# ecrireme/ESR-NeRF

Hardware: AMD Instinct MI355X
Metric: training rays/sec at 4096 rays x 128 samples (fine stage) (higher is better)
Workload: dtype f32; 1 GPU; C2: giftbox_w fine stage on the slab scene, 4096 rays x 128 samples per GPU, grid 256x256x64, s_val=20, forward + trainer loss + backward + the TV lines on every third step (no optimizer step); rays_per_gpu=4096, samples_per_ray=128, surviving_samples=524288, parallelism=dp1

## Files before the change

### esr_nerf_amd/_lib.py

```python
from __future__ import annotations

import ctypes as C
import os

import torch

_HERE = os.path.dirname(os.path.abspath(__file__))
LIB_PATH = os.path.join(_HERE, "libesr_hip.so")
LIB_PATH = os.environ.get("ESR_LIB_PATH", LIB_PATH)
ABI_VERSION = 30
_lib = None


class EsrScene(C.Structure):
    _fields_ = [
        ("xyz_min", C.c_float * 3), ("xyz_max", C.c_float * 3),
        ("mask_min", C.c_float * 3), ("mask_max", C.c_float * 3),
        ("gx", C.c_int32), ("gy", C.c_int32), ("gz", C.c_int32),
        ("mx", C.c_int32), ("my", C.c_int32), ("mz", C.c_int32),
        ("near_", C.c_float), ("stepdist", C.c_float), ("voxel_size", C.c_float),
        ("act_shift", C.c_float), ("mask_thres", C.c_float), ("fast_thres", C.c_float),
        ("s_val", C.c_float), ("max_steps", C.c_int32), ("grad_feat", C.c_float * 4),
    ]


class EsrPlan(C.Structure):
    _fields_ = [(n, C.c_int32) for n in
                ("n_on", "n_off", "tiles_on", "tiles_all", "m0", "m1", "m2", "overflow")]


class EsrFeatArgs(C.Structure):
    _fields_ = [(n, C.c_void_p) for n in ("rays_o", "rays_d", "viewdirs", "rec_ray", "rec_step", "rec_sdf",
                                          "pts", "pt_viewdirs", "pt_sdf")] + \
# ... 79 lines not shown
    _fields_ = [("w", C.c_void_p * 4), ("b", C.c_void_p * 4)]


class EsrWgradJob(C.Structure):
    _fields_ = [("kind", C.c_int32), ("color_row0", C.c_int32), ("t0", C.c_int32), ("t1", C.c_int32),
                ("X", C.c_void_p), ("H", C.c_void_p), ("dZ", C.c_void_p), ("dz", C.c_void_p),
                ("gw", C.c_void_p), ("gb", C.c_void_p), ("X16", C.c_void_p), ("amax", C.c_void_p)]


EXPORTS = [
    "esr_abi_version", "esr_build_info",
    "esr_sample_count", "esr_sample_fill", "esr_alpha2weight_fwd", "esr_alpha2weight_bwd",
    "esr_tv_add_grad", "esr_segment_sum",
    "esr_sample_count_f64", "esr_sample_fill_f64", "esr_alpha2weight_fwd_f64", "esr_alpha2weight_bwd_f64",
    "esr_infer_t_minmax", "esr_infer_n_samples", "esr_infer_ray_start_dir", "esr_sample_ndc_pts", "esr_sample_bg_pts",
    "esr_maskcache_lookup", "esr_raw2alpha", "esr_raw2alpha_bwd", "esr_tv_add_grad_masked",
    "esr_fine_march_count", "esr_fine_plan_begin", "esr_fine_plan", "esr_fine_plan_totals", "esr_fine_plan_offsets", "esr_fine_march_fill",
    "esr_fine_march_bwd", "esr_fine_march_bwd_rec", "esr_fine_march_cache_floats", "esr_fine_march_count_cached",
    "esr_fine_march_fill_cached", "esr_fine_march_bwd_cached", "esr_fine_march_count_ga", "esr_fine_march_fill_ga", "esr_fine_march_bwd_ga",
    "esr_fine_feat_fwd", "esr_fine_feat_fwd_x16", "esr_fine_feat_x16_bytes", "esr_fine_feat_bwd",
    "esr_mlp_packed_floats", "esr_mlp_pack", "esr_mlp_pack_batch", "esr_mlp_packed_split_elems", "esr_mlp_split_gain_offset", "esr_mlp_split_range_flag", "esr_mlp_fwd_split", "esr_mlp_fwd_fine_split", "esr_mlp_dgrad_split", "esr_mlp_dgrad_fine_split", "esr_absmax", "esr_mlp_fwd", "esr_mlp_fwd_mixed", "esr_mlp_fwd_fine", "esr_mlp_dgrad_fine", "esr_mlp_fwd_fine_bf16", "esr_mlp_dgrad_fine_bf16", "esr_mlp_dgrad", "esr_mlp_wgrad", "esr_mlp_wgrad_batch", "esr_tone_wgrad_scratch_floats", "esr_tone_wgrad_recompute", "esr_tone_wgrad_recompute_bf16", "esr_tone_wgrad_recompute_split",
    "esr_mlp_wgrad_scratch_floats",
    "esr_fine_tone_in_fwd", "esr_fine_composite_fwd", "esr_fine_composite_bwd",
    "esr_fine_tone_in_bwd", "esr_fine_loss_fwd_bwd_dp",
    "esr_expgrad_fwd", "esr_expgrad_bwd", "esr_lts_dirs", "esr_lts_ref_order", "esr_lts_perturb", "esr_lts_gather_rows",
    "esr_lts_gather_points", "esr_lts_combine_fwd", "esr_lts_combine_bwd",
    "esr_act_fwd", "esr_act_bwd", "esr_act_batch", "esr_lts_gather_rows_batch", "esr_pair_loss_batch", "esr_lts_ref_order_inv", "esr_lts_dirs_rays", "esr_composite3_fwd", "esr_composite3_bwd", "esr_lts_tone_in_bwd",
    "esr_sample_points", "esr_pair_loss_fwd_bwd", "esr_emit_edit",
    "esr_gauss3d_fwd", "esr_gauss3d_bwd", "esr_central_grad_fwd", "esr_central_grad_bwd",
    "esr_coarse_march_count", "esr_coarse_march_fill", "esr_coarse_march_bwd", "esr_coarse_march_count_ga", "esr_coarse_march_fill_ga", "esr_coarse_march_bwd_ga",
    "esr_coarse_feat_fwd", "esr_coarse_feat_bwd", "esr_coarse_shade_fwd", "esr_coarse_shade_bwd",
    "esr_adam_step", "esr_eval_aux", "esr_eval_disp",
    "esr_mlp_packed_bf16_elems", "esr_mlp_pack_bf16", "esr_mlp_fwd_bf16", "esr_mlp_dgrad_bf16", "esr_mlp_wgrad_bf16",
    "esr_brick_floats", "esr_brick_flags", "esr_brick_pack", "esr_brick_unpack", "esr_brick_list", "esr_brick_list_scratch_ints",
    "esr_smooth_grad_tv_fwd", "esr_smooth_grad_tv_bwd", "esr_host_choice_noreplace", "esr_host_choice_start", "esr_host_choice_wait",
    "esr_mesh_field", "esr_mesh_blocks", "esr_mesh_count", "esr_mesh_emit",
    "esr_cd_sample_count", "esr_cd_sample_fill", "esr_cd_cell_keys", "esr_cd_hash_insert", "esr_cd_downsample_round",
    "esr_cd_nn",
    "esr_dvgo_fwd", "esr_dvgo_eval", "esr_dvgo_bwd", "esr_dvgo_count", "esr_dvgo_count_add",
    "esr_ssim", "esr_view_post", "esr_sqerr_sum", "esr_gamma_curve", "esr_mask_iou",
    "esr_mask_dilate", "esr_edit_label",
]

SIGNATURES = {
    "esr_mask_dilate": (C.c_int, [C.c_void_p, C.c_int32, C.c_int32, C.c_int32, C.c_int32, C.c_void_p, C.c_void_p]),
    "esr_edit_label": (C.c_int, [C.c_void_p, C.c_int64, C.c_void_p, C.c_float, C.c_int32, C.c_int32, C.c_void_p, C.c_int32,
                                 C.c_void_p, C.c_void_p, C.c_void_p, C.c_void_p, C.c_void_p, C.c_void_p, C.c_void_p,
                                 C.c_void_p, C.c_void_p]),
}


def lib() -> C.CDLL:
    global _lib
    if _lib is None:
        if not os.path.exists(LIB_PATH):
            raise RuntimeError(
                f"{LIB_PATH} is missing: build it with `python -m esr_nerf_amd.build` "
                "(there is no CPU fallback for the HIP path)")
        L = C.CDLL(LIB_PATH)
        L.esr_abi_version.restype = C.c_int
        L.esr_build_info.restype = C.c_char_p
        if hasattr(L, "esr_mlp_packed_floats"):
            L.esr_mlp_packed_floats.restype = C.c_int64
            L.esr_mlp_wgrad_scratch_floats.restype = C.c_int64
            L.esr_tone_wgrad_scratch_floats.restype = C.c_int64
            L.esr_fine_march_cache_floats.restype = C.c_int64
        if hasattr(L, "esr_fine_feat_x16_bytes"):
            L.esr_fine_feat_x16_bytes.restype = C.c_int64
        if hasattr(L, "esr_brick_list_scratch_ints"):
            L.esr_brick_list_scratch_ints.restype = C.c_int64
        if hasattr(L, "esr_mlp_packed_bf16_elems"):
# ... 60 lines not shown
```

### esr_nerf_amd/csrc/shade.hip

```cpp
#include "esr_common.h"

namespace {

constexpr int XT_ROWS = 48;

__device__ __forceinline__ float softplus_grad(float z) { return z > 20.f ? 1.f : esr_sigmoid(z); }

__global__ void __launch_bounds__(256) tone_in_fwd_kernel(const float *__restrict__ z_off,
                                                          const float *__restrict__ z_emo, int tiles_on,
                                                          int tiles_all, float *__restrict__ lin,
                                                          float *__restrict__ Xt)
{
    const int total = tiles_all * 32;
    for (int j = blockIdx.x * blockDim.x + threadIdx.x; j < total; j += gridDim.x * blockDim.x) {
        const int t = j >> 5, s = j & 31;
        const size_t z4 = (size_t)t * 4 * 32 + s;
        float *X = Xt + (size_t)t * XT_ROWS * 32 + s;
#pragma unroll
        for (int c = 0; c < 3; ++c) {
            float v = esr_softplus(z_off[z4 + c * 32]);
            if (t < tiles_on) v = esr_softplus(z_emo[z4 + c * 32]) + v;
            lin[z4 + c * 32] = v;
            X[c * 32] = v;
#pragma unroll
// ... 109 lines not shown
            if (ray >= 0) {
                d = rec_w[j] * g_lin[3 * ray + c] + dX[c * 32];
#pragma unroll
                for (int i = 0; i < 5; ++i) {
                    const float f = (float)(1 << i);
                    d += f * (dX[(3 + c * 5 + i) * 32] * X[(18 + c * 5 + i) * 32] - dX[(18 + c * 5 + i) * 32] * X[(3 + c * 5 + i) * 32]);
                }
                const float z = (t < tiles_on) ? z_emo[z4 + c * 32] : z_off[z4 + c * 32];
                d *= softplus_grad(z);
            }
            dz[z4 + c * 32] = d;
        }
        dz[z4 + 96] = 0.f;
    }
}

__device__ __forceinline__ float wave_sum(float v)
{
#pragma unroll
    for (int off = 32; off > 0; off >>= 1) v += __shfl_xor(v, off);
    return v;
}

__global__ void __launch_bounds__(256) loss_kernel(const float *__restrict__ srgb_m,
                                                   const float *__restrict__ lin_m,
                                                   const float *__restrict__ last,
                                                   const float *__restrict__ rgbs, int n_rays, float white_bg,
                                                   float w_lin, float w_ent, float scale, float *__restrict__ loss,
                                                   float *__restrict__ g_srgb, float *__restrict__ g_lin,
                                                   float *__restrict__ g_last)
{
    const float inv = scale == 1.f ? 1.f / (3.f * (float)n_rays) : scale / (3.f * (float)n_rays);
    w_ent *= scale;
    float acc = 0.f;
    for (int r = blockIdx.x * blockDim.x + threadIdx.x; r < n_rays; r += gridDim.x * blockDim.x) {
        const float al = last[r];
        const float bg = al * white_bg;
        float gl = 0.f;
#pragma unroll
        for (int c = 0; c < 3; ++c) {
            const float gt = rgbs[3 * r + c];
            const float ps = srgb_m[3 * r + c] + bg;
            const float xs = fminf(fmaxf(ps, 0.f), 1.f);
            acc += (xs - gt) * (xs - gt) * inv;
            const float gs = (ps >= 0.f && ps <= 1.f) ? 2.f * (xs - gt) * inv : 0.f;
            g_srgb[3 * r + c] = gs;
            const float pl = lin_m[3 * r + c] + bg;
            const float l0 = fmaxf(pl, 0.f);
            const bool sat = gt >= 1.f;
            const float x = sat ? fminf(l0, 1.f) : l0;
            const bool low = x <= 0.0031308f;
            const float y = low ? 12.92f * x : 1.055f * powf(x, 1.f / 2.4f) - 0.055f;
            acc += w_lin * (y - gt) * (y - gt) * inv;
            float g = w_lin * 2.f * (y - gt) * inv;
            g *= low ? 12.92f : 1.055f * (1.f / 2.4f) * powf(x, 1.f / 2.4f - 1.f);
            if (sat && !(l0 <= 1.f)) g = 0.f;
            if (!(pl >= 0.f)) g = 0.f;
            g_lin[3 * r + c] = g;
            gl += (gs + g) * white_bg;
        }
        if (r == n_rays - 1) {
            const float p = fminf(fmaxf(al, 1e-6f), 1.f - 1e-6f);
            acc += w_ent * -(p * logf(p) + (1.f - p) * logf(1.f - p));
            if (al >= 1e-6f && al <= 1.f - 1e-6f) gl += w_ent * -(logf(p) - logf(1.f - p));
        }
        g_last[r] = gl;
    }
    acc = wave_sum(acc);
    if (esr_lane() == 0 && acc != 0.f) atomicAdd(loss, acc);
}

__global__ void __launch_bounds__(256) pair_loss_kernel(const float *__restrict__ a, const float *__restrict__ b,
                                                        int64_t rows, int cols, const uint8_t *__restrict__ row_mask,
                                                        int mask_value, const int32_t *__restrict__ count_dev, int kind,
                                                        float w_value, float w_a, float w_b, float *__restrict__ loss,
                                                        float *__restrict__ ga, float *__restrict__ gb)
{
    const int64_t total = rows * cols;
    const int64_t n_sel = count_dev ? (int64_t)count_dev[0] * cols : total;
    const float inv = n_sel > 0 ? 1.f / (float)n_sel : 0.f;
    float acc = 0.f;
    for (int64_t i = blockIdx.x * (int64_t)blockDim.x + threadIdx.x; i < total; i += (int64_t)gridDim.x * blockDim.x) {
        const bool sel = !row_mask || (int)row_mask[i / cols] == mask_value;
        float g = 0.f;
        if (sel) {
            const float d = a[i] - (b ? b[i] : 0.f);
            if (kind == 0) { acc += d * d * inv; g = 2.f * d * inv; }
            else { acc += fabsf(d) * inv; g = (d > 0.f ? 1.f : (d < 0.f ? -1.f : 0.f)) * inv; }
        }
        if (ga) ga[i] = w_a * g;
        if (gb) gb[i] = -w_b * g;
    }
// ... 292 lines not shown
    if (!dXt || !Xt || !g_lin || !lin || !z_off || (tiles_on && !z_emo) || !rec_ray || !rec_w || !dz) return ESR_EINVAL;
    tone_in_bwd_kernel<<<esr_grid_for((int64_t)tiles_all * 32, 256), 256, 0, esr_stream(stream)>>>(
        dXt, Xt, g_lin, lin, z_off, z_emo, rec_ray, rec_w, tiles_on, tiles_all, dz);
    ESR_CHECK_LAUNCH();
    return 0;
}

ESR_API int esr_fine_loss_fwd_bwd_dp(const float *srgb_marched, const float *lin_marched,
                                     const float *alphainv_last, const float *rgbs, int32_t n_rays,
                                     float white_bg, float weight_linear, float weight_entropy_last, float scale,
                                     float *loss, float *g_srgb, float *g_lin, float *g_last, void *stream)
{
    if (n_rays < 0) return ESR_EINVAL;
    if (n_rays == 0) return 0;
    if (!srgb_marched || !lin_marched || !alphainv_last || !rgbs || !loss || !g_srgb || !g_lin || !g_last)
        return ESR_EINVAL;
    loss_kernel<<<esr_grid_for(n_rays, 256), 256, 0, esr_stream(stream)>>>(
        srgb_marched, lin_marched, alphainv_last, rgbs, n_rays, white_bg, weight_linear,
        weight_entropy_last, scale, loss, g_srgb, g_lin, g_last);
    ESR_CHECK_LAUNCH();
    return 0;
}

ESR_API int esr_eval_aux(const float *X, int32_t xrows, int32_t row_nx, int32_t row_ny, int32_t row_nz,
                         const int32_t *rec_ray, const int32_t *rec_step, int32_t tiles,
                         const float *pos_rt_host, float stepdist, float *aux, void *stream)
{
    if (tiles < 0 || xrows < 1 || row_nx < 0 || row_ny < 0 || row_nz < 0 || row_nx >= xrows || row_ny >= xrows ||
        row_nz >= xrows)
        return ESR_EINVAL;
    if (tiles == 0) return 0;
    if (!X || !rec_ray || !rec_step || !pos_rt_host || !aux) return ESR_EINVAL;
    EvalAux A = {};
    A.X = X; A.rec_ray = rec_ray; A.rec_step = rec_step; A.tiles = tiles; A.xrows = xrows; A.stepdist = stepdist;
    A.aux = aux; A.nrow[0] = row_nx; A.nrow[1] = row_ny; A.nrow[2] = row_nz;
    for (int i = 0; i < 9; ++i) A.rt[i] = pos_rt_host[i];
    eval_aux_kernel<<<esr_grid_for((int64_t)tiles * 32, 256), 256, 0, esr_stream(stream)>>>(A);
    ESR_CHECK_LAUNCH();
    return 0;
}

ESR_API int esr_eval_disp(const float *depth3, const float *alphainv_last, float far_, int32_t n_rays,
                          float *depth, float *disp, void *stream)
{
    if (n_rays < 0) return ESR_EINVAL;
    if (n_rays == 0) return 0;
// ... 143 lines not shown
```

### esr_nerf_amd/fine_engine.py

```python
from __future__ import annotations

import ctypes as C
import functools
import math
import os
from dataclasses import dataclass
from typing import Dict, List, Optional

import torch

from . import _lib

KIND_RADIANCE, KIND_TONEMAP = 0, 1
HID = 192
X_ROWS, DX_ROWS, XT_ROWS = 104, 64, 48


def make_scene(xyz_min, xyz_max, mask_min, mask_max, world_size, mask_size, near, stepdist,
               voxel_size, act_shift, mask_thres, fast_thres, s_val, grad_feat) -> _lib.EsrScene:
    sc = _lib.EsrScene()
    for i in range(3):
        sc.xyz_min[i], sc.xyz_max[i] = float(xyz_min[i]), float(xyz_max[i])
        sc.mask_min[i], sc.mask_max[i] = float(mask_min[i]), float(mask_max[i])
    sc.gx, sc.gy, sc.gz = [int(v) for v in world_size]
# ... 20 lines not shown
    n: int
    rays_o: torch.Tensor
    rays_d: torch.Tensor
    viewdirs: Optional[torch.Tensor]
    mask_density: torch.Tensor
    sdf: torch.Tensor
    cnt3: torch.Tensor
    off3: torch.Tensor
    stats: torch.Tensor
    last: torch.Tensor
    cache: Optional[torch.Tensor] = None
    tiles_on: int = 0
    tiles_all: int = 0
    counts: Dict[str, int] = None
    e_pre: object = None


@dataclass
class FineCtx:
    march: March
    feat_args: object = None
    x16: bool = False
    f32_only: bool = False
    counts = property(lambda self: self.march.counts)


FINE_ROWS = dict(X=X_ROWS, gnorm=4, H0=HID, H1=HID, H2=HID, z_off=4, z_emo=4, lin=4, Xt=XT_ROWS, Ht=HID,
                 zt=4, rgb=4, dzt=4, dZt=HID, dXt=DX_ROWS, dz=4, dZ0=HID, dZ1=HID, dZ2=HID, dX=DX_ROWS,
                 dweight=1, rec_w=1, rec_sdf=1, dsdf=1)
FINE_OTHER = dict(M0=(192, torch.int32), M1=(192, torch.int32), M2=(192, torch.int32), Mt=(192, torch.int32),
                  rec_ray=(32, torch.int32), rec_step=(32, torch.int32), X16=(26 * 256, torch.uint8))


class _Workspace:
    min_tiles = 0

    def __init__(self, device, rows=FINE_ROWS, other=FINE_OTHER):
        self.device, self.rows, self.other = device, rows, other
        self.cap_tiles = 0
        self.buf: Dict[str, torch.Tensor] = {}
        self.ray_bufs: Dict[int, Dict[str, torch.Tensor]] = {}
        self.cache = None

    def ensure(self, tiles: int):
        if tiles <= self.cap_tiles:
            return
# ... 58 lines not shown

class FineEngine:
    def __init__(self, device, mlp_dtype: str = "f32"):
        if mlp_dtype not in ("f32", "bf16"):
            raise ValueError("mlp_dtype must be 'f32' or 'bf16'")
        self.device = torch.device(device)
        self.bf16 = mlp_dtype == "bf16"
        self.packed16: Dict[str, torch.Tensor] = {}
        self._p16: Dict[int, C.c_void_p] = {}
        self.L = _lib.lib()
        self.ws = _Workspace(self.device)
        self.plan_dev = torch.zeros(8, dtype=torch.int32, device=self.device)
        self.plan_host = torch.zeros(8, dtype=torch.int32).pin_memory()
        self.packed = {
            k: torch.empty(self.L.esr_mlp_packed_floats(kind), dtype=torch.float32, device=self.device)
            for k, kind in (("off", KIND_RADIANCE), ("emo", KIND_RADIANCE), ("tone", KIND_TONEMAP))}
        self.wgrad_scratch = torch.empty(self.L.esr_mlp_wgrad_scratch_floats(), dtype=torch.float32,
                                         device=self.device)
        self._timing = False
        self._only = None
        self._events = []
        self.n_calls = 0
        self.overlap_wgrad = True
        self._side = None
        self._raw: Dict[str, tuple] = {}
        self._pack_cache: Dict[str, tuple] = {}
        self._pack_pending = None
        self._pack_batch_cache = None
        self.x16 = self.bf16
        self.split_fwd = (not self.bf16) and os.environ.get("ESR_SPLIT_FWD", "1") != "0"
        self.split_strict = os.environ.get("ESR_SPLIT_STRICT", "0") == "1"
        self.split_fallback_steps = 0
        self.packed_split: Dict[str, torch.Tensor] = {}
        self._psplit = {}
        self.range_flag = None
        self._range_host = None
        self._range_event = None
        if self.split_fwd:
            key = str(self.device)
            if key not in _RANGE_FLAGS:
                _RANGE_FLAGS[key] = torch.zeros(1, dtype=torch.int32, device=self.device)
            self.range_flag = _RANGE_FLAGS[key]
            self._range_host = torch.zeros(1, dtype=torch.int32).pin_memory()
            with torch.cuda.device(self.device):
                _lib.check(self.L.esr_mlp_split_range_flag(_lib.ptr(self.range_flag)), "esr_mlp_split_range_flag")
        self.tone_scratch = torch.empty(self.L.esr_tone_wgrad_scratch_floats(), dtype=torch.float32, device=self.device)
# ... 263 lines not shown
        return _lib.ptr_array([self.ws[n] for n in names])

    def feat_args(self, m: March, rec, color_on, color_off):
        fa = _lib.EsrFeatArgs()
        fa.rays_o, fa.rays_d, fa.viewdirs = m.rays_o.data_ptr(), m.rays_d.data_ptr(), m.viewdirs.data_ptr()
        fa.rec_ray, fa.rec_step, fa.rec_sdf = rec[0].data_ptr(), rec[1].data_ptr(), rec[3].data_ptr()
        fa.sdf = m.sdf.data_ptr()
        for g in range(3):
            fa.color_on[g] = color_on[g].data_ptr() if color_on[g] is not None else None
            fa.color_off[g] = color_off[g].data_ptr() if color_off[g] is not None else None
        fa.tiles_on, fa.tiles_all = m.tiles_on, m.tiles_all
        return fa

    def _tone_wgrad(self, x, dz, t0, t1, gw, gb, amax, s, name):
        (w0, w1), (b0, _) = self._raw["tone"]
        L = self.L
        fn = L.esr_tone_wgrad_recompute_split if amax is not None else \
            L.esr_tone_wgrad_recompute_bf16 if self.bf16 else L.esr_tone_wgrad_recompute
        self._run(name, fn, _lib.ptr(x), _lib.ptr(dz), _lib.ptr(w0.detach()), _lib.ptr(b0.detach()), _lib.ptr(w1.detach()),
                  *((_lib.ptr(amax),) if amax is not None else ()), t0, t1, _lib.ptr(gw[0]), _lib.ptr(gb[0]), _lib.ptr(gw[1]),
                  _lib.ptr(gb[1]), _lib.ptr(self.tone_scratch), C.c_int64(self.tone_scratch.numel()), s)

    def forward(self, scene, rays_o, rays_d, viewdirs, em_modes, mask_density, sdf, off_color, emo_color, prelude=None,
                heal: bool = True):
        run = lambda: self._forward(scene, rays_o, rays_d, viewdirs, em_modes, mask_density, sdf, off_color, emo_color, prelude)
        return self.healed(run) if heal else run()

    def _forward(self, scene, rays_o, rays_d, viewdirs, em_modes, mask_density, sdf, off_color, emo_color, prelude=None):
        L, s, ws = self.L, self._s(), self.ws
        n = rays_o.shape[0]
        for t in (rays_o, rays_d, viewdirs):
            if t.dtype != torch.float32:
                raise RuntimeError("rays must be fp32")
        if em_modes.dtype != torch.int64:
            raise RuntimeError("em_modes must be int64")
        n3 = (3 * n + 3) // 4 * 4
        zb = torch.zeros(8 + 2 * n3 + 4, dtype=torch.float32, device=self.device)
        plan_dev = zb[:8].view(torch.int32)
        srgb, lin = zb[8: 8 + 3 * n].view(n, 3), zb[8 + n3: 8 + n3 + 3 * n].view(n, 3)
        self._loss_acc = zb[8 + 2 * n3: 8 + 2 * n3 + 2]
        self._amax = zb[8 + 2 * n3 + 3: 8 + 2 * n3 + 4]
        self._amax_t = zb[8 + 2 * n3 + 2: 8 + 2 * n3 + 3]
        sp = C.byref(scene)
        main = torch.cuda.current_stream(self.device)
        m = self._march_plan(ws, scene, rays_o, rays_d, viewdirs, em_modes, mask_density, sdf, plan_dev=plan_dev, prelude=prelude)
        last, e_pre, tiles_on, tiles_all = m.last, m.e_pre, m.tiles_on, m.tiles_all
        ctx = FineCtx(march=m, f32_only=not self.bf16 and not self.split_fwd)
        if tiles_all == 0:
            if e_pre is not None:
                main.wait_event(e_pre)
            self.range_probe()
# ... 8 lines not shown
        else:
            self._run("feat_fwd", L.esr_fine_feat_fwd, sp, C.byref(fa), _lib.ptr(ws["X"]), _lib.ptr(ws["gnorm"]), s)
        ctx.feat_args = fa
        H, M = self._H(["H0", "H1", "H2"]), self._H(["M0", "M1", "M2"])
        if e_pre is not None:
            main.wait_event(e_pre)
        if not self.bf16 and self.split_fwd and "off" in self.packed_split and "emo" in self.packed_split:
            self._run("mlp_fwd(rad)", L.esr_mlp_fwd_fine_split, _lib.ptr(self.packed["off"]), _lib.ptr(self.packed_split["off"]),
                      _lib.ptr(self.packed["emo"]), _lib.ptr(self.packed_split["emo"]), _lib.ptr(ws["X"]), tiles_on, tiles_all,
                      H, M, 88, _lib.ptr(ws["z_off"]), _lib.ptr(ws["z_emo"]), s)
        elif not self.bf16:
            self._run("mlp_fwd(rad)", L.esr_mlp_fwd_fine, _lib.ptr(self.packed["off"]), _lib.ptr(self.packed["emo"]),
                      _lib.ptr(ws["X"]), tiles_on, tiles_all, H, M, 88, _lib.ptr(ws["z_off"]), _lib.ptr(ws["z_emo"]), s)
        else:
            po, pe = _lib.ptr(self.packed["off"]), _lib.ptr(self.packed["emo"])
            self._run("mlp_fwd(rad)", L.esr_mlp_fwd_fine_bf16, po, self._p16[po.value], pe, self._p16[pe.value], _lib.ptr(ws["X"]),
                      _lib.ptr(ws["X16"]) if x16 else None, tiles_on, tiles_all, H, M, 88, _lib.ptr(ws["z_off"]),
                      _lib.ptr(ws["z_emo"]), s)
        self._run("tone_in_fwd", L.esr_fine_tone_in_fwd, _lib.ptr(ws["z_off"]), _lib.ptr(ws["z_emo"]), tiles_on, tiles_all,
                                          _lib.ptr(ws["lin"]), _lib.ptr(ws["Xt"]), s)
        self._run("mlp_fwd(tone)", self.mlp_fwd, KIND_TONEMAP, _lib.ptr(self.packed["tone"]), _lib.ptr(ws["Xt"]), 0, tiles_all,
                                 self._H(["Ht"]), self._H(["Mt"]), 2, 0, _lib.ptr(ws["zt"]), s)
        self.range_probe()
        self._run("composite_fwd", L.esr_fine_composite_fwd, _lib.ptr(ws["zt"]), _lib.ptr(ws["lin"]), _lib.ptr(ws["rec_ray"]),
                                            _lib.ptr(ws["rec_w"]), tiles_all, _lib.ptr(ws["rgb"]),
                                            _lib.ptr(srgb), _lib.ptr(lin), s)
        return ctx, last, srgb, lin

    @torch.no_grad()
    def evaluate(self, *args):
        return self.healed(lambda: self._evaluate(*args))

    def _evaluate(self, scene, rays_o, rays_d, viewdirs, mask_density, sdf, off_color, emo_color, pos_rt, far,
                  em_mode: int):
        L, s, ws, dev = self.L, self._s(), self.ws, self.device
        n = rays_o.shape[0]
        em0 = torch.zeros(n, dtype=torch.int64, device=dev)
        m = self._march_plan(ws, scene, rays_o, rays_d, viewdirs, em0, mask_density, sdf)
        T = m.tiles_all
        z3 = lambda: torch.zeros(n, 3, dtype=torch.float32, device=dev)
        out = {f"{sp_}/{v}_rgb": z3() for v in ("off", "on", "emo") for sp_ in ("srgb", "lin")}
        if T:
            sp = C.byref(scene)
            fa = self.feat_args(m, ws.rec(), color_on=(None, None, None), color_off=(off_color, emo_color, None))
            self._run("feat_fwd", L.esr_fine_feat_fwd, sp, C.byref(fa), _lib.ptr(ws["X"]), _lib.ptr(ws["gnorm"]), s)
            H, M = self._H(["H0", "H1", "H2"]), self._H(["M0", "M1", "M2"])
# ... 78 lines not shown
            todo = [(KIND_RADIANCE, ws["X"], Hh, dZh, ws["dz"], 0, to, "emo_w", "emo_b"),
                    (KIND_RADIANCE, ws["X"], Hh, dZh, ws["dz"], to, ta, "off_w", "off_b")]
            jobs = (_lib.EsrWgradJob * len(todo))()
            for j, (kind, X, Hs, dZs, dzs, r0, r1, gwk, gbk) in enumerate(todo):
                gwa, gba = _lib.ptr_array(grads[gwk]), _lib.ptr_array(grads[gbk])
                keep += [gwa, gba]
                jb = jobs[j]
                jb.kind, jb.color_row0, jb.t0, jb.t1 = kind, 0, r0, r1
                jb.X, jb.dz = X.data_ptr(), dzs.data_ptr()
                jb.H, jb.dZ = C.addressof(Hs), C.addressof(dZs)
                jb.gw, jb.gb = C.addressof(gwa), C.addressof(gba)
                if ctx.x16:
                    jb.X16 = ws["X16"].data_ptr()
                if split:
                    jb.amax = ctx.amax.data_ptr()
            self._run("mlp_wgrad(all)", L.esr_mlp_wgrad_batch, jobs, len(todo), 1 if self.bf16 else 0,
                      _lib.ptr(self.wgrad_scratch), C.c_int64(self.wgrad_scratch.numel()), s_)

        if ta == 0:
            march_bwd(s)
            if after_grids is not None:
                after_grids()
            return
        self._run("composite_bwd", L.esr_fine_composite_bwd, _lib.ptr(g_srgb), _lib.ptr(g_lin), _lib.ptr(ws["rgb"]),
                  _lib.ptr(ws["lin"]), _lib.ptr(ws["rec_ray"]), _lib.ptr(ws["rec_w"]), ta, _lib.ptr(ws["dweight"]),
                  _lib.ptr(ws["dzt"]), s)
        if fold:
            march_bwd(s)
        dZt_arg = _lib.ptr_array([None])
        M = self._H(["M0", "M1", "M2"])
        dZ = self._H(["dZ0", "dZ1", "dZ2"])
        if self.bf16:
            self._run("mlp_dgrad(tone)", L.esr_mlp_dgrad_bf16, KIND_TONEMAP, self._p16[self.packed["tone"].data_ptr()],
                      _lib.ptr(ws["dzt"]), 0, ta, self._H(["Mt"]), dZt_arg, _lib.ptr(ws["dXt"]), s)
        elif split:
            self._run("mlp_dgrad(tone)", L.esr_mlp_dgrad_split, KIND_TONEMAP, _lib.ptr(self.packed_split["tone"]), _lib.ptr(ws["dzt"]),
                      0, ta, self._H(["Mt"]), dZt_arg, _lib.ptr(ws["dXt"]), _lib.ptr(ctx.amax_t), s)
        else:
            self._run("mlp_dgrad(tone)", L.esr_mlp_dgrad, KIND_TONEMAP, _lib.ptr(self.packed["tone"]), _lib.ptr(ws["dzt"]), 0, ta,
                      self._H(["Mt"]), dZt_arg, _lib.ptr(ws["dXt"]), s)
        self._run("tone_in_bwd", L.esr_fine_tone_in_bwd, _lib.ptr(ws["dXt"]), _lib.ptr(ws["Xt"]), _lib.ptr(g_lin), _lib.ptr(ws["lin"]),
                  _lib.ptr(ws["z_off"]), _lib.ptr(ws["z_emo"]), _lib.ptr(ws["rec_ray"]), _lib.ptr(ws["rec_w"]), to, ta,
                  _lib.ptr(ws["dz"]), s)
        if self.bf16:
            pe, po = self.packed["emo"].data_ptr(), self.packed["off"].data_ptr()
            self._run("mlp_dgrad(rad)", L.esr_mlp_dgrad_fine_bf16, self._p16[pe], self._p16[po],
                      _lib.ptr(ws["dz"]), to, ta, M, dZ, _lib.ptr(ws["dX"]), s)
        elif split:
            self._run("mlp_dgrad(rad)", L.esr_mlp_dgrad_fine_split, _lib.ptr(self.packed_split["emo"]),
                      _lib.ptr(self.packed_split["off"]), _lib.ptr(ws["dz"]), to, ta, M, dZ, _lib.ptr(ws["dX"]),
                      _lib.ptr(ctx.amax), s)
        else:
            self._run("mlp_dgrad(rad)", L.esr_mlp_dgrad_fine, _lib.ptr(self.packed["emo"]), _lib.ptr(self.packed["off"]),
                      _lib.ptr(ws["dz"]), to, ta, M, dZ, _lib.ptr(ws["dX"]), s)
        if not overlap:
            feat_bwd(s)
            if not fold:
                march_bwd(s)
            if after_grids is not None:
                after_grids()
            wgrads(s)
            return
        e_dgrad = torch.cuda.Event()
        e_dgrad.record(main)
        side = self._side_stream(0)
        side.wait_event(e_dgrad)
        with torch.cuda.stream(side):
            wgrads(_lib.stream_ptr(self.device))
            e_w = torch.cuda.Event()
            e_w.record(side)
        feat_bwd(s)
        if not fold:
            march_bwd(s)
        if after_grids is not None:
            after_grids()
        main.wait_event(e_w)

    def _side_stream(self, i=0):
        if self._side is None:
            self._side = {}
        if i not in self._side:
            self._side[i] = torch.cuda.Stream(self.device)
        return self._side[i]

    def loss_fwd_bwd(self, last, srgb, lin, rgbs, white_bg=True, weight_linear=0.1, weight_entropy_last=0.001,
                     scale=1.0):
        n = last.shape[0]
        acc = getattr(self, "_loss_acc", None)
        self._loss_acc = None
        pair = acc if acc is not None and acc.device == srgb.device else torch.zeros(2, dtype=torch.float32, device=self.device)
        self.loss_pair = pair
        loss = pair[:1]
        g_srgb = torch.empty_like(srgb)
        g_lin = torch.empty_like(lin)
        g_last = torch.empty_like(last)
        self._run("loss", self.L.esr_fine_loss_fwd_bwd_dp,
                  _lib.ptr(srgb), _lib.ptr(lin), _lib.ptr(last), _lib.ptr(rgbs.contiguous()), n,
                  C.c_float(1.0 if white_bg else 0.0), C.c_float(weight_linear), C.c_float(weight_entropy_last),
                  C.c_float(scale), _lib.ptr(loss), _lib.ptr(g_srgb), _lib.ptr(g_lin), _lib.ptr(g_last), self._s())
        return loss, g_last, g_srgb, g_lin
```

### esr_nerf_amd/trainer.py

```python
from __future__ import annotations

import os

from typing import Dict, Optional, Tuple

import torch

from .fine_engine import KIND_RADIANCE, KIND_TONEMAP


def shard_batch(batch: Dict[str, torch.Tensor], rank: int, world: int) -> Dict[str, torch.Tensor]:
    n = next(iter(batch.values())).shape[0]
    per = n // world
    lo = rank * per
    hi = n if rank == world - 1 else lo + per
    return {k: v[lo:hi].contiguous() for k, v in batch.items()}


def dp_loss_weights(n_local: int, global_rays, entropy_owner: bool, weight_entropy_last: float):
    scale = 1.0 if global_rays is None else n_local / float(global_rays)
    w_ent = (weight_entropy_last / scale) if entropy_owner else 0.0
    return scale, w_ent


# ... 250 lines not shown
                              global_rays: Optional[int] = None,
                              entropy_owner: bool = True,
                              regularisers: Optional[dict] = None) -> Tuple[torch.Tensor, Dict[str, torch.Tensor]]:
        m = self.model
        eng = m.engine
        m.s_val = s_val
        ps = m._mlp_params()
        return self._step(eng, lambda _: self._attempt(batch, global_rays, entropy_owner, m, eng, ps, regularisers))

    def _attempt(self, batch, global_rays, entropy_owner, m, eng, ps, regularisers):
        g = None

        def prelude():
            nonlocal g
            with eng.packing():
                eng.pack("off", KIND_RADIANCE, list(ps[0:8:2]), list(ps[1:8:2]))
                eng.pack("emo", KIND_RADIANCE, list(ps[8:16:2]), list(ps[9:16:2]))
                eng.pack("tone", KIND_TONEMAP, list(ps[16:20:2]), list(ps[17:20:2]))
            g = self._alloc_grads(batch["rays_o"].device)

        ctx, last, srgb, lin = eng.forward(
            m.scene_struct(), batch["rays_o"], batch["rays_d"], batch["viewdirs"], batch["em_modes"],
            m.mask_cache.density.view(*m.mask_cache.density.shape[2:]),
            m.sdf.device_view(), m.off_color.device_view(), m.emo_color.device_view(), prelude=prelude, heal=False)
        m.last_counts = ctx.counts
        if self.pg is not None:
            self._check_overflow()
        scale, w_ent = dp_loss_weights(last.shape[0], global_rays, entropy_owner, self.weight_entropy_last)
        loss, g_last, g_srgb, g_lin = eng.loss_fwd_bwd(last, srgb, lin, batch["rgbs"], self.white_bg,
                                                       self.weight_linear, w_ent, scale=scale)
        names = self._param_names()
        grads = dict(sdf=g["sdf.grid"], off_color=g["off_color.grid"], emo_color=g["emo_color.grid"],
                     off_w=[g[n] for n in names[0:8:2]], off_b=[g[n] for n in names[1:8:2]],
                     emo_w=[g[n] for n in names[8:16:2]], emo_b=[g[n] for n in names[9:16:2]],
                     tone_w=[g[n] for n in names[16:20:2]], tone_b=[g[n] for n in names[17:20:2]])
        loss = self._backward(eng, lambda after_grids: eng.backward(ctx, g_last, g_srgb, g_lin, grads, after_grids=after_grids),
                              loss, g, regularisers)
        return None if loss is None else (loss, self._handout(g))


class LtsStep(_Step):

    GRIDS = FineStep.GRIDS + ("brdf",)
    NETS = FineStep.NETS + (("brdfnet", "brdfnet"), ("emitnet", "brdfnet"))
    TAIL = ("envmap.mus", "envmap.lambdas", "envmap.lobes")

    def __init__(self, model, trainer_cfg, stage: str = "lts", white_bg: bool = True, process_group=None,
                 split_points: bool = False):
        if stage not in ("lts", "pdra"):
            raise ValueError("stage must be 'lts' or 'pdra'")
        super().__init__(model, process_group)
        self.t, self.stage, self.white_bg = trainer_cfg, stage, white_bg
        self.ltspts = int(model.num_ltspts)
# ... 127 lines not shown
```

### include/esr_hip.h

```cpp
#ifndef ESR_HIP_H
#define ESR_HIP_H

#include <stdint.h>

#ifdef __cplusplus
extern "C" {
#endif

#define ESR_EINVAL (-1)
#define ESR_ECAP   (-2)

#define ESR_TILE 32

#define ESR_ABI_VERSION 30
int esr_abi_version(void);
const char *esr_build_info(void);


int esr_sample_count(const float *rays_o, const float *rays_d, const float *xyz_min,
                     const float *xyz_max, float near_, float far_, float stepdist,
                     int64_t n_rays, float *t_min, float *t_max, int64_t *n_steps,
                     int64_t *cumsum, int64_t *total, void *stream);

int esr_sample_fill(const float *rays_o, const float *rays_d, const float *xyz_min,
                    const float *xyz_max, const float *t_min, const int64_t *cumsum,
                    float stepdist, int64_t n_rays, int64_t total, float *ray_pts,
                    uint8_t *mask_outbbox, int64_t *ray_id, int64_t *step_id, void *stream);

int esr_alpha2weight_fwd(const float *alpha, const int64_t *ray_id, int64_t n_pts,
                         int64_t n_rays, float *weight, float *T, float *alphainv_last,
                         int64_t *i_start, int64_t *i_end, void *stream);

int esr_alpha2weight_bwd(const float *alpha, const float *weight, const float *T,
                         const float *alphainv_last, const int64_t *i_start,
                         const int64_t *i_end, int64_t n_pts, int64_t n_rays,
                         const float *grad_weights, const float *grad_last, float *grad,
                         void *stream);
// ... 233 lines not shown
                       void *stream);

int esr_fine_tone_in_fwd(const float *z_off, const float *z_emo, int32_t tiles_on,
                         int32_t tiles_all, float *lin, float *Xt, void *stream);

int esr_fine_composite_fwd(const float *zt, const float *lin, const int32_t *rec_ray,
                           const float *rec_w, int32_t tiles_all, float *rgb,
                           float *srgb_marched, float *lin_marched, void *stream);

int esr_fine_composite_bwd(const float *g_srgb, const float *g_lin, const float *rgb,
                           const float *lin, const int32_t *rec_ray, const float *rec_w,
                           int32_t tiles_all, float *dweight, float *dzt, void *stream);

int esr_fine_tone_in_bwd(const float *dXt, const float *Xt, const float *g_lin, const float *lin,
                         const float *z_off, const float *z_emo, const int32_t *rec_ray,
                         const float *rec_w, int32_t tiles_on, int32_t tiles_all, float *dz,
                         void *stream);

int esr_fine_loss_fwd_bwd_dp(const float *srgb_marched, const float *lin_marched,
                             const float *alphainv_last, const float *rgbs, int32_t n_rays,
                             float white_bg, float weight_linear, float weight_entropy_last, float scale,
                             float *loss, float *g_srgb, float *g_lin, float *g_last,
                             void *stream);

int esr_pair_loss_fwd_bwd(const float *a, const float *b, int64_t rows, int32_t cols,
                          const uint8_t *row_mask, int mask_value, const int32_t *count_dev,
                          int kind, float w_value, float w_a, float w_b, float *loss, float *ga,
                          float *gb, void *stream);


int esr_expgrad_fwd(const esr_scene_t *scene, const float *rays_o, const float *rays_d,
                    const int32_t *rec_ray, const int32_t *rec_step, const float *pts,
                    const float *noise, float eps, const float *sdf, int32_t n, int zero_pad,
                    float *out, void *stream);
int esr_expgrad_bwd(const esr_scene_t *scene, const float *rays_o, const float *rays_d,
                    const int32_t *rec_ray, const int32_t *rec_step, const float *pts,
                    const float *noise, float eps, const float *g, int32_t n, int zero_pad,
                    float *grad_sdf, void *stream);

int esr_lts_ref_order(const int32_t *rec_ray, const int32_t *cnt3, const int32_t *off3, const int64_t *cnt3_cumsum,
                      int32_t n_slots, int64_t *perm, int64_t *ray64, void *stream);
int esr_lts_perturb(const float *pts_all, const int64_t *perm, const float *noise_normal, const float *noise_emit,
                    float emit_eps, int32_t m3, float *noise_n, float *pts_e, void *stream);
int esr_lts_gather_rows(const float *src, int32_t tile_rows, int32_t row_stride, int32_t col0, int32_t n_ch,
                        const int64_t *perm, int32_t n, float *out, void *stream);
typedef struct esr_lts_gather {
// ... 317 lines not shown
```

Before: 2.045 million rays/s.

## Fuse fine composite, loss and composite backward into one per-ray kernel

Adds a shade_loss kernel that, with one wavefront per ray, composites the sigmoid colours and linear values, evaluates the photometric and entropy loss and gradients, and writes dzt and dweight in a single launch. This replaces the separate composite_fwd, loss and composite_bwd kernels along with their intermediate rgb buffer traffic. It also moves march backward onto a side stream so it can overlap with the remaining backward work. The cost is redundant sigmoid and global reads for rays with more than 128 samples, plus extra stream and event synchronisation.

```diff
diff --git a/esr_nerf_amd/_lib.py b/esr_nerf_amd/_lib.py
--- a/esr_nerf_amd/_lib.py
+++ b/esr_nerf_amd/_lib.py
@@ -8,7 +8,7 @@
 _HERE = os.path.dirname(os.path.abspath(__file__))
 LIB_PATH = os.path.join(_HERE, "libesr_hip.so")
 LIB_PATH = os.environ.get("ESR_LIB_PATH", LIB_PATH)
-ABI_VERSION = 30
+ABI_VERSION = 31
 _lib = None
 
 
@@ -134,7 +134,7 @@
     "esr_mlp_packed_floats", "esr_mlp_pack", "esr_mlp_pack_batch", "esr_mlp_packed_split_elems", "esr_mlp_split_gain_offset", "esr_mlp_split_range_flag", "esr_mlp_fwd_split", "esr_mlp_fwd_fine_split", "esr_mlp_dgrad_split", "esr_mlp_dgrad_fine_split", "esr_absmax", "esr_mlp_fwd", "esr_mlp_fwd_mixed", "esr_mlp_fwd_fine", "esr_mlp_dgrad_fine", "esr_mlp_fwd_fine_bf16", "esr_mlp_dgrad_fine_bf16", "esr_mlp_dgrad", "esr_mlp_wgrad", "esr_mlp_wgrad_batch", "esr_tone_wgrad_scratch_floats", "esr_tone_wgrad_recompute", "esr_tone_wgrad_recompute_bf16", "esr_tone_wgrad_recompute_split",
     "esr_mlp_wgrad_scratch_floats",
     "esr_fine_tone_in_fwd", "esr_fine_composite_fwd", "esr_fine_composite_bwd",
-    "esr_fine_tone_in_bwd", "esr_fine_loss_fwd_bwd_dp",
+    "esr_fine_tone_in_bwd", "esr_fine_loss_fwd_bwd_dp", "esr_fine_shade_loss",
     "esr_expgrad_fwd", "esr_expgrad_bwd", "esr_lts_dirs", "esr_lts_ref_order", "esr_lts_perturb", "esr_lts_gather_rows",
     "esr_lts_gather_points", "esr_lts_combine_fwd", "esr_lts_combine_bwd",
     "esr_act_fwd", "esr_act_bwd", "esr_act_batch", "esr_lts_gather_rows_batch", "esr_pair_loss_batch", "esr_lts_ref_order_inv", "esr_lts_dirs_rays", "esr_composite3_fwd", "esr_composite3_bwd", "esr_lts_tone_in_bwd",
@@ -159,6 +159,7 @@
     "esr_edit_label": (C.c_int, [C.c_void_p, C.c_int64, C.c_void_p, C.c_float, C.c_int32, C.c_int32, C.c_void_p, C.c_int32,
                                  C.c_void_p, C.c_void_p, C.c_void_p, C.c_void_p, C.c_void_p, C.c_void_p, C.c_void_p,
                                  C.c_void_p, C.c_void_p]),
+    "esr_fine_shade_loss": (C.c_int, [C.c_void_p] * 7 + [C.c_int32] * 5 + [C.c_float] * 4 + [C.c_void_p] * 9),
 }
 
 
diff --git a/esr_nerf_amd/csrc/shade.hip b/esr_nerf_amd/csrc/shade.hip
--- a/esr_nerf_amd/csrc/shade.hip
+++ b/esr_nerf_amd/csrc/shade.hip
@@ -155,6 +155,31 @@
     return v;
 }
 
+__device__ __forceinline__ float loss_channel(float ps, float pl, float gt, float inv, float w_lin, float &gs, float &g)
+{
+    const float xs = fminf(fmaxf(ps, 0.f), 1.f);
+    float acc = (xs - gt) * (xs - gt) * inv;
+    gs = (ps >= 0.f && ps <= 1.f) ? 2.f * (xs - gt) * inv : 0.f;
+    const float l0 = fmaxf(pl, 0.f);
+    const bool sat = gt >= 1.f;
+    const float x = sat ? fminf(l0, 1.f) : l0;
+    const bool low = x <= 0.0031308f;
+    const float y = low ? 12.92f * x : 1.055f * powf(x, 1.f / 2.4f) - 0.055f;
+    acc += w_lin * (y - gt) * (y - gt) * inv;
+    g = w_lin * 2.f * (y - gt) * inv;
+    g *= low ? 12.92f : 1.055f * (1.f / 2.4f) * powf(x, 1.f / 2.4f - 1.f);
+    if (sat && !(l0 <= 1.f)) g = 0.f;
+    if (!(pl >= 0.f)) g = 0.f;
+    return acc;
+}
+
+__device__ __forceinline__ float loss_entropy_last(float al, float w_ent, float &gl)
+{
+    const float p = fminf(fmaxf(al, 1e-6f), 1.f - 1e-6f);
+    if (al >= 1e-6f && al <= 1.f - 1e-6f) gl += w_ent * -(logf(p) - logf(1.f - p));
+    return w_ent * -(p * logf(p) + (1.f - p) * logf(1.f - p));
+}
+
 __global__ void __launch_bounds__(256) loss_kernel(const float *__restrict__ srgb_m,
                                                    const float *__restrict__ lin_m,
                                                    const float *__restrict__ last,
@@ -172,35 +197,136 @@
         float gl = 0.f;
 #pragma unroll
         for (int c = 0; c < 3; ++c) {
-            const float gt = rgbs[3 * r + c];
-            const float ps = srgb_m[3 * r + c] + bg;
-            const float xs = fminf(fmaxf(ps, 0.f), 1.f);
-            acc += (xs - gt) * (xs - gt) * inv;
-            const float gs = (ps >= 0.f && ps <= 1.f) ? 2.f * (xs - gt) * inv : 0.f;
+            float gs, g;
+            acc += loss_channel(srgb_m[3 * r + c] + bg, lin_m[3 * r + c] + bg, rgbs[3 * r + c], inv, w_lin, gs, g);
             g_srgb[3 * r + c] = gs;
-            const float pl = lin_m[3 * r + c] + bg;
-            const float l0 = fmaxf(pl, 0.f);
-            const bool sat = gt >= 1.f;
-            const float x = sat ? fminf(l0, 1.f) : l0;
-            const bool low = x <= 0.0031308f;
-            const float y = low ? 12.92f * x : 1.055f * powf(x, 1.f / 2.4f) - 0.055f;
-            acc += w_lin * (y - gt) * (y - gt) * inv;
-            float g = w_lin * 2.f * (y - gt) * inv;
-            g *= low ? 12.92f : 1.055f * (1.f / 2.4f) * powf(x, 1.f / 2.4f - 1.f);
-            if (sat && !(l0 <= 1.f)) g = 0.f;
-            if (!(pl >= 0.f)) g = 0.f;
             g_lin[3 * r + c] = g;
             gl += (gs + g) * white_bg;
         }
-        if (r == n_rays - 1) {
-            const float p = fminf(fmaxf(al, 1e-6f), 1.f - 1e-6f);
-            acc += w_ent * -(p * logf(p) + (1.f - p) * logf(1.f - p));
-            if (al >= 1e-6f && al <= 1.f - 1e-6f) gl += w_ent * -(logf(p) - logf(1.f - p));
-        }
+        if (r == n_rays - 1) acc += loss_entropy_last(al, w_ent, gl);
         g_last[r] = gl;
     }
     acc = wave_sum(acc);
     if (esr_lane() == 0 && acc != 0.f) atomicAdd(loss, acc);
+}
+
+constexpr int SL_KEEP = 2;
+struct ShadeLoss {
+    const float *zt, *lin, *rec_w;
+    const int32_t *off3, *cnt3;
+    const float *last, *rgbs;
+    int n_rays, n_on, n_off, tiles_on, tiles_all;
+    float white_bg, w_lin, w_ent, scale;
+    float *loss, *srgb_m, *lin_m, *g_srgb, *g_lin, *g_last, *dzt, *dweight;
+};
+__global__ void __launch_bounds__(1024) shade_loss_kernel(ShadeLoss A)
+{
+    __shared__ float part[16];
+    const int lane = esr_lane();
+    const int wv = __builtin_amdgcn_readfirstlane((int)(threadIdx.x >> 6)), nwv = (int)(blockDim.x >> 6);
+    const int total = A.tiles_all * 32;
+    const float inv = A.scale == 1.f ? 1.f / (3.f * (float)A.n_rays) : A.scale / (3.f * (float)A.n_rays);
+    const float w_ent = A.w_ent * A.scale;
+    if (blockIdx.x == 0 && wv == 0) {
+        const bool on = lane < 32;
+        const int j = (on ? A.n_on : A.tiles_on * 32 + A.n_off) + (lane & 31);
+        if (j < (on ? A.tiles_on * 32 : total)) {
+            const size_t z4 = (size_t)(j >> 5) * 4 * 32 + (j & 31);
+#pragma unroll
+            for (int c = 0; c < 4; ++c) A.dzt[z4 + c * 32] = 0.f;
+            A.dweight[j] = 0.f;
+        }
+    }
+    float acc = 0.f;
+    for (int r = blockIdx.x * nwv + wv; r < A.n_rays; r += gridDim.x * nwv) {
+        const int off_r = A.off3[r], cnt = A.cnt3[r];
+        const bool any = off_r >= 0 && cnt > 0 && off_r < total;
+        const int off = any ? off_r : 0, end = any ? (cnt < total - off ? off + cnt : total) : 0;
+        const float al = A.last[r];
+        const float gt = A.rgbs[3 * r + (lane < 3 ? lane : 0)];
+        float col[SL_KEEP][3], l[SL_KEEP][3], w[SL_KEEP];
+        float sum[6] = {0.f, 0.f, 0.f, 0.f, 0.f, 0.f};
+#pragma unroll
+        for (int k = 0; k < SL_KEEP; ++k) {
+            const int j = off + k * 64 + lane;
+            const bool ok = j < end;
+            const size_t z4 = (size_t)(j >> 5) * 4 * 32 + (j & 31);
+            w[k] = ok ? A.rec_w[j] : 0.f;
+#pragma unroll
+            for (int c = 0; c < 3; ++c) {
+                col[k][c] = ok ? esr_sigmoid(A.zt[z4 + c * 32]) : 0.f;
+                l[k][c] = ok ? A.lin[z4 + c * 32] : 0.f;
+                sum[c] += w[k] * col[k][c];
+                sum[3 + c] += w[k] * l[k][c];
+            }
+        }
+        for (int j = off + SL_KEEP * 64 + lane; j < end; j += 64) {
+            const size_t z4 = (size_t)(j >> 5) * 4 * 32 + (j & 31);
+            const float wj = A.rec_w[j];
+#pragma unroll
+            for (int c = 0; c < 3; ++c) {
+                sum[c] += wj * esr_sigmoid(A.zt[z4 + c * 32]);
+                sum[3 + c] += wj * A.lin[z4 + c * 32];
+            }
+        }
+#pragma unroll
+        for (int i = 0; i < 6; ++i) sum[i] = wave_sum(sum[i]);
+        const float bg = al * A.white_bg;
+        const float sm = lane == 0 ? sum[0] : lane == 1 ? sum[1] : sum[2];
+        const float lm = lane == 0 ? sum[3] : lane == 1 ? sum[4] : sum[5];
+        float gs_c, g_c;
+        const float a_c = loss_channel(sm + bg, lm + bg, gt, inv, A.w_lin, gs_c, g_c);
+        if (lane < 3) {
+            acc += a_c;
+            A.srgb_m[3 * r + lane] = sm;
+            A.lin_m[3 * r + lane] = lm;
+            A.g_srgb[3 * r + lane] = gs_c;
+            A.g_lin[3 * r + lane] = g_c;
+        }
+        float gs[3], g[3], gl = 0.f;
+#pragma unroll
+        for (int c = 0; c < 3; ++c) {
+            gs[c] = esr_readlane(gs_c, c);
+            g[c] = esr_readlane(g_c, c);
+            gl += (gs[c] + g[c]) * A.white_bg;
+        }
+        if (r == A.n_rays - 1) {
+            const float e = loss_entropy_last(al, w_ent, gl);
+            if (lane == 0) acc += e;
+        }
+        if (lane == 0) A.g_last[r] = gl;
+        auto bwd = [&](int j, float wj, const float *cj, const float *lj) {
+            const size_t z4 = (size_t)(j >> 5) * 4 * 32 + (j & 31);
+            float dw = 0.f;
+#pragma unroll
+            for (int c = 0; c < 3; ++c) {
+                dw += gs[c] * cj[c] + g[c] * lj[c];
+                A.dzt[z4 + c * 32] = wj * gs[c] * cj[c] * (1.f - cj[c]);
+            }
+            A.dzt[z4 + 96] = 0.f;
+            A.dweight[j] = dw;
+        };
+#pragma unroll
+        for (int k = 0; k < SL_KEEP; ++k) {
+            const int j = off + k * 64 + lane;
+            if (j < end) bwd(j, w[k], col[k], l[k]);
+        }
+        for (int j = off + SL_KEEP * 64 + lane; j < end; j += 64) {
+            const size_t z4 = (size_t)(j >> 5) * 4 * 32 + (j & 31);
+            float cj[3], lj[3];
+#pragma unroll
+            for (int c = 0; c < 3; ++c) { cj[c] = esr_sigmoid(A.zt[z4 + c * 32]); lj[c] = A.lin[z4 + c * 32]; }
+            bwd(j, A.rec_w[j], cj, lj);
+        }
+    }
+    acc = wave_sum(acc);
+    if (lane == 0) part[wv] = acc;
+    __syncthreads();
+    if (threadIdx.x == 0) {
+        float tot = 0.f;
+        for (int i = 0; i < nwv; ++i) tot += part[i];
+        if (tot != 0.f) atomicAdd(A.loss, tot);
+    }
 }
 
 __global__ void __launch_bounds__(256) pair_loss_kernel(const float *__restrict__ a, const float *__restrict__ b,
@@ -539,6 +665,30 @@
     return 0;
 }
 
+ESR_API int esr_fine_shade_loss(const float *zt, const float *lin, const float *rec_w, const int32_t *off3,
+                                const int32_t *cnt3, const float *alphainv_last, const float *rgbs, int32_t n_rays,
+                                int32_t n_on, int32_t n_off, int32_t tiles_on, int32_t tiles_all, float white_bg,
+                                float weight_linear, float weight_entropy_last, float scale, float *loss,
+                                float *srgb_marched, float *lin_marched, float *g_srgb, float *g_lin, float *g_last,
+                                float *dzt, float *dweight, void *stream)
+{
+    if (n_rays < 0 || n_on < 0 || n_off < 0 || tiles_on != (n_on + 31) / 32 || tiles_all - tiles_on != (n_off + 31) / 32)
+        return ESR_EINVAL;
+    if (n_rays == 0) return tiles_all ? ESR_EINVAL : 0;
+    if (!off3 || !cnt3 || !alphainv_last || !rgbs || !loss || !srgb_marched || !lin_marched || !g_srgb || !g_lin || !g_last)
+        return ESR_EINVAL;
+    if (tiles_all && (!zt || !lin || !rec_w || !dzt || !dweight)) return ESR_EINVAL;
+    ShadeLoss A = {};
+    A.zt = zt; A.lin = lin; A.rec_w = rec_w; A.off3 = off3; A.cnt3 = cnt3; A.last = alphainv_last; A.rgbs = rgbs;
+    A.n_rays = n_rays; A.n_on = n_on; A.n_off = n_off; A.tiles_on = tiles_on; A.tiles_all = tiles_all;
+    A.white_bg = white_bg; A.w_lin = weight_linear; A.w_ent = weight_entropy_last; A.scale = scale;
+    A.loss = loss; A.srgb_m = srgb_marched; A.lin_m = lin_marched; A.g_srgb = g_srgb; A.g_lin = g_lin; A.g_last = g_last;
+    A.dzt = dzt; A.dweight = dweight;
+    shade_loss_kernel<<<esr_grid_for(n_rays, 16, 256 * 8), 1024, 0, esr_stream(stream)>>>(A);
+    ESR_CHECK_LAUNCH();
+    return 0;
+}
+
 ESR_API int esr_eval_aux(const float *X, int32_t xrows, int32_t row_nx, int32_t row_ny, int32_t row_nz,
                          const int32_t *rec_ray, const int32_t *rec_step, int32_t tiles,
                          const float *pos_rt_host, float stepdist, float *aux, void *stream)
diff --git a/esr_nerf_amd/fine_engine.py b/esr_nerf_amd/fine_engine.py
--- a/esr_nerf_amd/fine_engine.py
+++ b/esr_nerf_amd/fine_engine.py
@@ -66,6 +66,7 @@
     feat_args: object = None
     x16: bool = False
     f32_only: bool = False
+    shaded: bool = False
     counts = property(lambda self: self.march.counts)
 
 
@@ -170,6 +171,8 @@
         self._events = []
         self.n_calls = 0
         self.overlap_wgrad = True
+        self.fused_shade = True
+        self.march_bwd_side = True
         self._side = None
         self._raw: Dict[str, tuple] = {}
         self._pack_cache: Dict[str, tuple] = {}
@@ -479,11 +482,13 @@
                   _lib.ptr(gb[1]), _lib.ptr(self.tone_scratch), C.c_int64(self.tone_scratch.numel()), s)
 
     def forward(self, scene, rays_o, rays_d, viewdirs, em_modes, mask_density, sdf, off_color, emo_color, prelude=None,
-                heal: bool = True):
-        run = lambda: self._forward(scene, rays_o, rays_d, viewdirs, em_modes, mask_density, sdf, off_color, emo_color, prelude)
+                heal: bool = True, composite: bool = True):
+        run = lambda: self._forward(scene, rays_o, rays_d, viewdirs, em_modes, mask_density, sdf, off_color, emo_color, prelude,
+                                    composite)
         return self.healed(run) if heal else run()
 
-    def _forward(self, scene, rays_o, rays_d, viewdirs, em_modes, mask_density, sdf, off_color, emo_color, prelude=None):
+    def _forward(self, scene, rays_o, rays_d, viewdirs, em_modes, mask_density, sdf, off_color, emo_color, prelude=None,
+                 composite=True):
         L, s, ws = self.L, self._s(), self.ws
         n = rays_o.shape[0]
         for t in (rays_o, rays_d, viewdirs):
@@ -538,6 +543,8 @@
         self._run("mlp_fwd(tone)", self.mlp_fwd, KIND_TONEMAP, _lib.ptr(self.packed["tone"]), _lib.ptr(ws["Xt"]), 0, tiles_all,
                                  self._H(["Ht"]), self._H(["Mt"]), 2, 0, _lib.ptr(ws["zt"]), s)
         self.range_probe()
+        if not composite:
+            return ctx, last, srgb, lin
         self._run("composite_fwd", L.esr_fine_composite_fwd, _lib.ptr(ws["zt"]), _lib.ptr(ws["lin"]), _lib.ptr(ws["rec_ray"]),
                                             _lib.ptr(ws["rec_w"]), tiles_all, _lib.ptr(ws["rgb"]),
                                             _lib.ptr(srgb), _lib.ptr(lin), s)
@@ -662,10 +669,21 @@
             if after_grids is not None:
                 after_grids()
             return
-        self._run("composite_bwd", L.esr_fine_composite_bwd, _lib.ptr(g_srgb), _lib.ptr(g_lin), _lib.ptr(ws["rgb"]),
-                  _lib.ptr(ws["lin"]), _lib.ptr(ws["rec_ray"]), _lib.ptr(ws["rec_w"]), ta, _lib.ptr(ws["dweight"]),
-                  _lib.ptr(ws["dzt"]), s)
-        if fold:
+        if not ctx.shaded:
+            self._run("composite_bwd", L.esr_fine_composite_bwd, _lib.ptr(g_srgb), _lib.ptr(g_lin), _lib.ptr(ws["rgb"]),
+                      _lib.ptr(ws["lin"]), _lib.ptr(ws["rec_ray"]), _lib.ptr(ws["rec_w"]), ta, _lib.ptr(ws["dweight"]),
+                      _lib.ptr(ws["dzt"]), s)
+        e_march = None
+        if fold and overlap and self.march_bwd_side:
+            e_shade = torch.cuda.Event()
+            e_shade.record(main)
+            side = self._side_stream(0)
+            side.wait_event(e_shade)
+            with torch.cuda.stream(side):
+                march_bwd(_lib.stream_ptr(self.device))
+                e_march = torch.cuda.Event()
+                e_march.record(side)
+        elif fold:
             march_bwd(s)
         dZt_arg = _lib.ptr_array([None])
         M = self._H(["M0", "M1", "M2"])
@@ -709,6 +727,8 @@
             wgrads(_lib.stream_ptr(self.device))
             e_w = torch.cuda.Event()
             e_w.record(side)
+        if e_march is not None:
+            main.wait_event(e_march)
         feat_bwd(s)
         if not fold:
             march_bwd(s)
@@ -723,19 +743,32 @@
             self._side[i] = torch.cuda.Stream(self.device)
         return self._side[i]
 
-    def loss_fwd_bwd(self, last, srgb, lin, rgbs, white_bg=True, weight_linear=0.1, weight_entropy_last=0.001,
-                     scale=1.0):
-        n = last.shape[0]
+    def _loss_bufs(self, last, srgb, lin):
         acc = getattr(self, "_loss_acc", None)
         self._loss_acc = None
         pair = acc if acc is not None and acc.device == srgb.device else torch.zeros(2, dtype=torch.float32, device=self.device)
         self.loss_pair = pair
-        loss = pair[:1]
-        g_srgb = torch.empty_like(srgb)
-        g_lin = torch.empty_like(lin)
-        g_last = torch.empty_like(last)
+        return pair[:1], torch.empty_like(last), torch.empty_like(srgb), torch.empty_like(lin)
+
+    def loss_fwd_bwd(self, last, srgb, lin, rgbs, white_bg=True, weight_linear=0.1, weight_entropy_last=0.001,
+                     scale=1.0):
+        n = last.shape[0]
+        loss, g_last, g_srgb, g_lin = self._loss_bufs(last, srgb, lin)
         self._run("loss", self.L.esr_fine_loss_fwd_bwd_dp,
                   _lib.ptr(srgb), _lib.ptr(lin), _lib.ptr(last), _lib.ptr(rgbs.contiguous()), n,
                   C.c_float(1.0 if white_bg else 0.0), C.c_float(weight_linear), C.c_float(weight_entropy_last),
                   C.c_float(scale), _lib.ptr(loss), _lib.ptr(g_srgb), _lib.ptr(g_lin), _lib.ptr(g_last), self._s())
         return loss, g_last, g_srgb, g_lin
+
+    def shade_loss(self, ctx: FineCtx, last, srgb, lin, rgbs, white_bg=True, weight_linear=0.1, weight_entropy_last=0.001,
+                   scale=1.0):
+        m, ws = ctx.march, self.ws
+        loss, g_last, g_srgb, g_lin = self._loss_bufs(last, srgb, lin)
+        T = m.tiles_all
+        tile = (lambda k: _lib.ptr(ws[k])) if T else (lambda k: None)
+        self._run("shade_loss", self.L.esr_fine_shade_loss, tile("zt"), tile("lin"), tile("rec_w"), _lib.ptr(m.off3), _lib.ptr(m.cnt3),
+                  _lib.ptr(last), _lib.ptr(rgbs.contiguous()), m.n, m.counts["n_on"], m.counts["n_off"], m.tiles_on, T,
+                  1.0 if white_bg else 0.0, weight_linear, weight_entropy_last, scale, _lib.ptr(loss), _lib.ptr(srgb),
+                  _lib.ptr(lin), _lib.ptr(g_srgb), _lib.ptr(g_lin), _lib.ptr(g_last), tile("dzt"), tile("dweight"), self._s())
+        ctx.shaded = True
+        return loss, g_last, g_srgb, g_lin
diff --git a/esr_nerf_amd/trainer.py b/esr_nerf_amd/trainer.py
--- a/esr_nerf_amd/trainer.py
+++ b/esr_nerf_amd/trainer.py
@@ -296,13 +296,18 @@
         ctx, last, srgb, lin = eng.forward(
             m.scene_struct(), batch["rays_o"], batch["rays_d"], batch["viewdirs"], batch["em_modes"],
             m.mask_cache.density.view(*m.mask_cache.density.shape[2:]),
-            m.sdf.device_view(), m.off_color.device_view(), m.emo_color.device_view(), prelude=prelude, heal=False)
+            m.sdf.device_view(), m.off_color.device_view(), m.emo_color.device_view(), prelude=prelude, heal=False,
+            composite=not eng.fused_shade)
         m.last_counts = ctx.counts
         if self.pg is not None:
             self._check_overflow()
         scale, w_ent = dp_loss_weights(last.shape[0], global_rays, entropy_owner, self.weight_entropy_last)
-        loss, g_last, g_srgb, g_lin = eng.loss_fwd_bwd(last, srgb, lin, batch["rgbs"], self.white_bg,
-                                                       self.weight_linear, w_ent, scale=scale)
+        if eng.fused_shade:
+            loss, g_last, g_srgb, g_lin = eng.shade_loss(ctx, last, srgb, lin, batch["rgbs"], self.white_bg,
+                                                         self.weight_linear, w_ent, scale=scale)
+        else:
+            loss, g_last, g_srgb, g_lin = eng.loss_fwd_bwd(last, srgb, lin, batch["rgbs"], self.white_bg,
+                                                           self.weight_linear, w_ent, scale=scale)
         names = self._param_names()
         grads = dict(sdf=g["sdf.grid"], off_color=g["off_color.grid"], emo_color=g["emo_color.grid"],
                      off_w=[g[n] for n in names[0:8:2]], off_b=[g[n] for n in names[1:8:2]],
diff --git a/include/esr_hip.h b/include/esr_hip.h
--- a/include/esr_hip.h
+++ b/include/esr_hip.h
@@ -12,7 +12,7 @@
 
 #define ESR_TILE 32
 
-#define ESR_ABI_VERSION 30
+#define ESR_ABI_VERSION 31
 int esr_abi_version(void);
 const char *esr_build_info(void);
 
@@ -292,6 +292,14 @@
                              float white_bg, float weight_linear, float weight_entropy_last, float scale,
                              float *loss, float *g_srgb, float *g_lin, float *g_last,
                              void *stream);
+
+int esr_fine_shade_loss(const float *zt, const float *lin, const float *rec_w, const int32_t *off3,
+                        const int32_t *cnt3, const float *alphainv_last, const float *rgbs,
+                        int32_t n_rays, int32_t n_on, int32_t n_off, int32_t tiles_on,
+                        int32_t tiles_all, float white_bg, float weight_linear,
+                        float weight_entropy_last, float scale, float *loss, float *srgb_marched,
+                        float *lin_marched, float *g_srgb, float *g_lin, float *g_last, float *dzt,
+                        float *dweight, void *stream);
 
 int esr_pair_loss_fwd_bwd(const float *a, const float *b, int64_t rows, int32_t cols,
                           const uint8_t *row_mask, int mask_value, const int32_t *count_dev,
```

Result: no change. 2.033 million rays/s (-0.6%).
